# parsakhaz/multimodal-image-similarity-search

Hardware: AMD Instinct MI355X
Metric: images/s CLIP-B/32 encode @ bs256; Mvec/s cosine top-10 over 10M x 512 (higher is better)
Workload: dtype bf16

## Files before the change

multimodal-image-similarity-search_amd/csrc/gemm_bf16_p160.h:

```cpp
#pragma once
#include "gemm_bf16_256.h"

#define G160_A_BYTES 20480
#define G160_W_BYTES 16384
#define G160_BUF (G160_A_BYTES + 2 * G160_W_BYTES)
#define G160_DUMP (3 * G160_BUF)
#define G160_LDS (G160_DUMP + 2048)

template <int EPI, int KT = 0>
__global__ __launch_bounds__(512, 2) void gemm160p_kernel(const __bf16* __restrict__ A, const __bf16* __restrict__ W, int M,
                                                          int N, int K, GemmEpi ep) {
    extern __shared__ __attribute__((aligned(16))) char smem[];
    typedef bf16x8 frag;
    const int tid = threadIdx.x;
    const int lane = tid & 63;
    const int wave = __builtin_amdgcn_readfirstlane(tid >> 6);
    const int wm = wave >> 2, wn = wave & 3;
    const int fr = lane & 15, fg = lane >> 4;
    const int nbm = M / 160, nbn = N >> 8;
    const int nt = KT > 0 ? KT : K / GEMM_BK;
    const int wg = xcd_remap(blockIdx.x, nbm * nbn);
    int bm, bn;
    tile_order(wg, nbm, nbn, 0, bm, bn);
    const __bf16* Ab = A + (size_t)bm * 160 * K;
    const __bf16* Wb = W + (size_t)bn * 256 * K;

    const int r_in = lane >> 3, p = lane & 7;
    const int lane_vo = (r_in * K + ((p ^ r_in) * 8)) * 2;
    const __amdgpu_buffer_rsrc_t srdA = __builtin_amdgcn_make_buffer_rsrc(const_cast<__bf16*>(Ab), 0, 0x7fffffff, 0x00020000);
    const __amdgpu_buffer_rsrc_t srdW = __builtin_amdgcn_make_buffer_rsrc(const_cast<__bf16*>(Wb), 0, 0x7fffffff, 0x00020000);
    const int row8 = 8 * K * 2;
    const int a_so = wave * row8;
    const int a_dst = wave * 1024;
    const int w_so = ((wave >> 1) * 64 + (wave & 1) * 16) * K * 2;
    const int w_dst = wave * 2048;
    char* const dump = smem + G160_DUMP + wave * 256;
#define G160_BLDS(srd, so, dst) \
    __builtin_amdgcn_raw_ptr_buffer_load_lds(srd, (__attribute__((address_space(3))) void*)(dst), 16, lane_vo, so, 0, 0)
#define G160_FILL(srd, so) \
    __builtin_amdgcn_raw_ptr_buffer_load_lds(srd, (__attribute__((address_space(3))) void*)(dump), 4, lane_vo, so, 0, 0)
#define G160_STAGE_A(b2, ko)                                                                                 \
    {                                                                                                       \
        char* sl_ = smem + (b2) * G160_BUF + a_dst;                                                         \
        G160_BLDS(srdA, a_so + (ko), sl_);                                                                  \
        G160_BLDS(srdA, a_so + 8 * row8 + (ko), sl_ + 8 * 1024);                                            \
        if (wave < 4) { G160_BLDS(srdA, a_so + 16 * row8 + (ko), sl_ + 16 * 1024); }                        \
        else { G160_FILL(srdA, a_so + (ko)); }                                                              \
    }
#define G160_STAGE_W(b2, nq, ko)                                                                             \
    {                                                                                                       \
        char* sl_ = smem + (b2) * G160_BUF + G160_A_BYTES + (nq) * G160_W_BYTES + w_dst;                    \
        const int so_ = w_so + (nq) * 4 * row8 + (ko);                                                      \
        G160_BLDS(srdW, so_, sl_);                                                                          \
        G160_BLDS(srdW, so_ + row8, sl_ + 1024);                                                            \
    }

    uint32_t ab[2], wb[2];
#pragma unroll
    for (int s = 0; s < 2; ++s) {
        const uint32_t sw = (((4 * s + fg) ^ (fr & 7)) << 4);
        ab[s] = (wm * 80 + fr) * 128 + sw;
        wb[s] = G160_A_BYTES + (wn * 32 + fr) * 128 + sw;
    }
    frag am[5];
    frag wq[4];
    f32x4 acc[4][5];
#pragma unroll
    for (int i = 0; i < 4; ++i)
#pragma unroll
        for (int j = 0; j < 5; ++j) acc[i][j] = f32x4{0.f, 0.f, 0.f, 0.f};

#define G160_READ(b, s)                                                                                      \
    {                                                                                                       \
        _Pragma("unroll") for (int mf = 0; mf < 5; ++mf)                                                    \
            am[mf] = *reinterpret_cast<const frag*>(smem + ab[s] + (b) * G160_BUF + mf * 2048);             \
        _Pragma("unroll") for (int i = 0; i < 4; ++i)                                                       \
            wq[i] = *reinterpret_cast<const frag*>(smem + wb[s] + (b) * G160_BUF + (i >> 1) * G160_W_BYTES + (i & 1) * 2048); \
    }
#define G160_MMA()                                                                                           \
    {                                                                                                       \
        __builtin_amdgcn_s_setprio(1);                                                                      \
        _Pragma("unroll") for (int i = 0; i < 4; ++i)                                                       \
            _Pragma("unroll") for (int mf = 0; mf < 5; ++mf)                                                \
                acc[i][mf] = __builtin_amdgcn_mfma_f32_16x16x32_bf16(wq[i], am[mf], acc[i][mf], 0, 0, 0);   \
        __builtin_amdgcn_s_setprio(0);                                                                      \
    }
#define G160_BARRIER()                            \
    {                                             \
        __builtin_amdgcn_sched_barrier(0);        \
        __builtin_amdgcn_s_barrier();             \
        __builtin_amdgcn_sched_barrier(0);        \
    }
#define G160_LATE_READS_DONE() \
    if (wm == 1) asm volatile("s_waitcnt lgkmcnt(0)" ::: "memory")
#define G160_KTILE(B, B2)                                                                                    \
    {                                                                                                       \
        G160_READ(B, 0);                                                                                    \
        G160_STAGE_A(B2, ko2);                                                                              \
        G160_LATE_READS_DONE();                                                                             \
        G160_BARRIER();                                                                                     \
        G160_MMA();                                                                                         \
        G160_BARRIER();                                                                                     \
        G160_READ(B, 1);                                                                                    \
        G160_STAGE_W(B2, 0, ko2);                                                                           \
        G160_STAGE_W(B2, 1, ko2);                                                                           \
        G160_LATE_READS_DONE();                                                                             \
        asm volatile("s_waitcnt vmcnt(7)" ::: "memory");                                                    \
        G160_BARRIER();                                                                                     \
        G160_MMA();                                                                                         \
        G160_BARRIER();                                                                                     \
        if (++k2 == nt) { k2 = 0; ko2 = 0; } else { ko2 += GEMM_BK * 2; }                                   \
    }

    constexpr bool RESID = (EPI == MMISS_EPI_BIAS_RESID_BF16);
    static_assert(RESID || EPI == MMISS_EPI_PATCH_F32, "gemm160p_kernel: epilogue");
    u32x2 resid[5][4];
    f32x4 bias[4];
    if constexpr (RESID) {
        const uint16_t* ob = reinterpret_cast<const uint16_t*>(ep.out) + (size_t)(bm * 160 + wm * 80 + fr) * ep.ldo + bn * 256 + wn * 64 + 4 * fg;
#pragma unroll
        for (int j = 0; j < 5; ++j)
#pragma unroll
            for (int i = 0; i < 4; ++i) resid[j][i] = *reinterpret_cast<const u32x2*>(ob + (size_t)j * 16 * ep.ldo + i * 16);
#pragma unroll
        for (int i = 0; i < 4; ++i) bias[i] = *reinterpret_cast<const f32x4*>(ep.bias + bn * 256 + wn * 64 + i * 16 + 4 * fg);
    }

    int ko2 = 0, k2 = 2;
    G160_STAGE_A(0, 0);
    G160_STAGE_W(0, 0, 0);
    G160_STAGE_W(0, 1, 0);
    G160_STAGE_A(1, GEMM_BK * 2);
    G160_STAGE_W(1, 0, GEMM_BK * 2);
    G160_STAGE_W(1, 1, GEMM_BK * 2);
    ko2 = (nt > 2) ? 2 * GEMM_BK * 2 : 0;
    asm volatile("s_waitcnt vmcnt(7)" ::: "memory");
    if constexpr (RESID) {
#pragma unroll
        for (int j = 0; j < 5; ++j)
#pragma unroll
            for (int i = 0; i < 4; ++i) asm volatile("" : "+v"(resid[j][i]));
#pragma unroll
        for (int i = 0; i < 4; ++i) asm volatile("" : "+v"(bias[i]));
    }
    G160_BARRIER();
    if (wm == 1) G160_BARRIER();

#pragma unroll 1
    for (int t = 0; t < nt; t += 3) {
        G160_KTILE(0, 2);
        if (t + 1 < nt) G160_KTILE(1, 0);
        if (t + 2 < nt) G160_KTILE(2, 1);
    }
    if (wm == 0) G160_BARRIER();
    asm volatile("s_waitcnt vmcnt(0)" ::: "memory");
    G160_BARRIER();

    if constexpr (EPI == MMISS_EPI_PATCH_F32) {
        int lane_e = lane;
        asm volatile("" : "+v"(lane_e));
        const int efr = lane_e & 15, efg = lane_e >> 4;
        const int rrow = lane_e >> 3, rchunk = lane_e & 7;
        char* patch = smem + wave * 2048;
        float* outp = reinterpret_cast<float*>(ep.out);
#pragma unroll
        for (int j = 0; j < 5; ++j) {
#pragma unroll
            for (int h = 0; h < 2; ++h) {
#pragma unroll
                for (int ii = 0; ii < 2; ++ii)
                    *reinterpret_cast<f32x4*>(patch + efr * 128 + (((ii * 4 + efg) ^ (efr & 7)) << 4)) = acc[2 * h + ii][j];
                __builtin_amdgcn_fence(__ATOMIC_RELEASE, "wavefront");
                __builtin_amdgcn_wave_barrier();
                __builtin_amdgcn_fence(__ATOMIC_ACQUIRE, "wavefront");
#pragma unroll
                for (int rh = 0; rh < 2; ++rh) {
                    const int row = rh * 8 + rrow;
                    const f32x4 v = *reinterpret_cast<const f32x4*>(patch + row * 128 + ((rchunk ^ (row & 7)) << 4));
                    const int m = bm * 160 + wm * 80 + j * 16 + row;
                    const int n = bn * 256 + wn * 64 + h * 32 + rchunk * 4;
                    if (m < ep.m_valid) {
                        const int img = m / ep.p0, pt = m - img * ep.p0;
                        const f32x4 pos = *reinterpret_cast<const f32x4*>(ep.aux + (size_t)(1 + pt) * ep.ldo + n);
                        *reinterpret_cast<f32x4*>(outp + ((size_t)img * ep.p1 + 1 + pt) * ep.ldo + n) = v + pos;
                    }
                }
                __builtin_amdgcn_wave_barrier();
            }
        }
    }
    if constexpr (RESID) {
        int lane_e = lane;
        asm volatile("" : "+v"(lane_e));
        const int efr = lane_e & 15, efg = lane_e >> 4;
        const int rrow = lane_e >> 3, rchunk = lane_e & 7;
        const __amdgpu_buffer_rsrc_t srdO = __builtin_amdgcn_make_buffer_rsrc(ep.out, 0, 0x7fffffff, 0x00020000);
        char* patch = smem + wave * 2048;
        const int wr_off = efr * 128, wr_sw = 2 * (efr & 7);
        const int col = bn * 256 + wn * 64 + rchunk * 8;
        const int dump_row = M - 1;
#pragma unroll
        for (int j = 0; j < 5; ++j) {
#pragma unroll
            for (int i = 0; i < 4; ++i) {
                const f32x4 v = acc[i][j] + bias[i];
                float y[4];
                y[0] = __uint_as_float(resid[j][i][0] << 16) + v[0];
                y[1] = __uint_as_float(resid[j][i][0] & 0xFFFF0000u) + v[1];
                y[2] = __uint_as_float(resid[j][i][1] << 16) + v[2];
                y[3] = __uint_as_float(resid[j][i][1] & 0xFFFF0000u) + v[3];
                u32x2 pk;
                pk[0] = pack_bf16x2(y[0], y[1]);
                pk[1] = pack_bf16x2(y[2], y[3]);
                *reinterpret_cast<u32x2*>(patch + wr_off + (((i * 4 + efg) ^ wr_sw) << 3)) = pk;
            }
            __builtin_amdgcn_fence(__ATOMIC_RELEASE, "wavefront");
            __builtin_amdgcn_wave_barrier();
            __builtin_amdgcn_fence(__ATOMIC_ACQUIRE, "wavefront");
#pragma unroll
            for (int rh = 0; rh < 2; ++rh) {
                const int row = rh * 8 + rrow;
                const u32x4 pk = *reinterpret_cast<const u32x4*>(patch + row * 128 + (((2 * rchunk) ^ (2 * (row & 7))) << 3));
                const int m = bm * 160 + wm * 80 + j * 16 + row;
                const int vo = ((m < ep.m_valid ? m : dump_row) * ep.ldo + col) * 2;
                __builtin_amdgcn_raw_buffer_store_b128(pk, srdO, vo, 0, 0);
                if (ep.stats_out) {
                    float rs = 0.f, rq = 0.f;
#pragma unroll
                    for (int e = 0; e < 4; ++e) {
                        const float a = __uint_as_float(pk[e] << 16), b = __uint_as_float(pk[e] & 0xFFFF0000u);
                        rs += a + b;
                        rq += a * a + b * b;
                    }
                    rs += __shfl_xor(rs, 1); rq += __shfl_xor(rq, 1);
                    rs += __shfl_xor(rs, 2); rq += __shfl_xor(rq, 2);
                    rs += __shfl_xor(rs, 4); rq += __shfl_xor(rq, 4);
                    if (rchunk == 0 && m < ep.m_valid) {
                        float* so = ep.stats_out + ((size_t)m * (ep.ldo >> 6) + ((bn * 256 + wn * 64) >> 6)) * 2;
                        so[0] = rs;
                        so[1] = rq;
                    }
                }
            }
            __builtin_amdgcn_wave_barrier();
        }
    }
}
#undef G160_BLDS
#undef G160_FILL
#undef G160_STAGE_A
#undef G160_STAGE_W
#undef G160_READ
#undef G160_MMA
#undef G160_BARRIER
#undef G160_LATE_READS_DONE
#undef G160_KTILE

static inline bool gemm160p_ok(int M, int N, int K) {
    if (M <= 0 || (M % 160) || N <= 0 || (N % 256) || K < 256 || (K % 128)) return false;
    if ((int64_t)M * N * 2 >= (1LL << 31) || (int64_t)160 * K * 2 >= (1LL << 31) || (int64_t)256 * K * 2 >= (1LL << 31)) return false;
    return true;
}

static int launch_gemm160p(hipStream_t st, const void* A, const void* W, const GemmEpi& ep, int M, int N, int K) {
    if (!gemm160p_ok(M, N, K)) MM_FAIL(MMISS_ERR_UNSUPPORTED, "gemm160p: M=%d N=%d K=%d", M, N, K);
    if (!ep.out || !ep.bias || ep.ldo < N || (ep.ldo % 64)) MM_FAIL(MMISS_ERR_ARG, "gemm160p: missing operand");
    const int mv = ep.m_valid < M ? ep.m_valid : M;
    const double bytes = 2.0 * ((double)mv * K + (double)N * K) + 2.0 * 2.0 * (double)mv * N;
    char pname[48];
    snprintf(pname, sizeof(pname), "gemm_bf16_bias_resid16_p160_k%d", K);
    MM_PROF(pname, st, 2.0 * mv * N * K, bytes);
#define G160_KT_CASE(KT_)                                                                                                        \
    if (K == (KT_) * GEMM_BK) {                                                                                                  \
        MM_TRY(mmiss_ensure_dyn_lds(reinterpret_cast<const void*>(&gemm160p_kernel<MMISS_EPI_BIAS_RESID_BF16, KT_>), G160_LDS)); \
        hipLaunchKernelGGL((gemm160p_kernel<MMISS_EPI_BIAS_RESID_BF16, KT_>), dim3((M / 160) * (N / 256)), dim3(512), G160_LDS, \
                           st, reinterpret_cast<const __bf16*>(A), reinterpret_cast<const __bf16*>(W), M, N, K, ep);            \
        MM_HIP(hipGetLastError());                                                                                              \
        return MMISS_OK;                                                                                                        \
    }
    G160_KT_CASE(12) G160_KT_CASE(48) G160_KT_CASE(8) G160_KT_CASE(32) G160_KT_CASE(16) G160_KT_CASE(64)
#undef G160_KT_CASE
    MM_TRY(mmiss_ensure_dyn_lds(reinterpret_cast<const void*>(&gemm160p_kernel<MMISS_EPI_BIAS_RESID_BF16>), G160_LDS));
    hipLaunchKernelGGL((gemm160p_kernel<MMISS_EPI_BIAS_RESID_BF16>), dim3((M / 160) * (N / 256)), dim3(512), G160_LDS, st, reinterpret_cast<const __bf16*>(A),
                       reinterpret_cast<const __bf16*>(W), M, N, K, ep);
    MM_HIP(hipGetLastError());
    return MMISS_OK;
}

static int launch_gemm160p_patch(hipStream_t st, const void* A, const void* W, const GemmEpi& ep, int M, int N, int K) {
    if (!gemm160p_ok(M, N, K)) MM_FAIL(MMISS_ERR_UNSUPPORTED, "gemm160p_patch: M=%d N=%d K=%d", M, N, K);
    if (!ep.out || !ep.aux || ep.p0 <= 0 || ep.p1 <= 0 || ep.ldo < N) MM_FAIL(MMISS_ERR_ARG, "gemm160p_patch: missing operand");
    const int mv = ep.m_valid < M ? ep.m_valid : M;
    MM_PROF("gemm_bf16_patch_p160", st, 2.0 * mv * N * K, 2.0 * ((double)mv * K + (double)N * K) + 4.0 * (double)mv * N);
    MM_TRY(mmiss_ensure_dyn_lds(reinterpret_cast<const void*>(&gemm160p_kernel<MMISS_EPI_PATCH_F32>), G160_LDS));
    hipLaunchKernelGGL((gemm160p_kernel<MMISS_EPI_PATCH_F32>), dim3((M / 160) * (N / 256)), dim3(512), G160_LDS, st,
                       reinterpret_cast<const __bf16*>(A), reinterpret_cast<const __bf16*>(W), M, N, K, ep);
    MM_HIP(hipGetLastError());
    return MMISS_OK;
}
```

Measured before the change: 89280.

## Prefetch residual tile via pipelined buffer loads into LDS instead of registers

Instead of loading the bf16 residual tile into VGPRs before the main loop, the last two pipeline prefetch slots are repurposed. Once the K loop wraps, the buffer resources and offsets are retargeted at the output residual rows, so the residual streams into the spare LDS stage buffers via buffer_load_lds. The epilogue then reads the residual from LDS and uses a free stage buffer for its patch staging. This removes 40 held registers across the main loop and overlaps the residual fetch with compute, at the cost of more complex offset bookkeeping and a tight coupling to the 3-stage buffer indexing.

```diff
diff --git a/multimodal-image-similarity-search_amd/csrc/gemm_bf16_p160.h b/multimodal-image-similarity-search_amd/csrc/gemm_bf16_p160.h
--- a/multimodal-image-similarity-search_amd/csrc/gemm_bf16_p160.h
+++ b/multimodal-image-similarity-search_amd/csrc/gemm_bf16_p160.h
@@ -25,15 +25,21 @@
     const __bf16* Ab = A + (size_t)bm * 160 * K;
     const __bf16* Wb = W + (size_t)bn * 256 * K;
 
+    constexpr bool RESID = (EPI == MMISS_EPI_BIAS_RESID_BF16);
+    static_assert(RESID || EPI == MMISS_EPI_PATCH_F32, "gemm160p_kernel: epilogue");
     const int r_in = lane >> 3, p = lane & 7;
-    const int lane_vo = (r_in * K + ((p ^ r_in) * 8)) * 2;
-    const __amdgpu_buffer_rsrc_t srdA = __builtin_amdgcn_make_buffer_rsrc(const_cast<__bf16*>(Ab), 0, 0x7fffffff, 0x00020000);
-    const __amdgpu_buffer_rsrc_t srdW = __builtin_amdgcn_make_buffer_rsrc(const_cast<__bf16*>(Wb), 0, 0x7fffffff, 0x00020000);
+    int lane_vo = (r_in * K + ((p ^ r_in) * 8)) * 2;
+    __amdgpu_buffer_rsrc_t srdA = __builtin_amdgcn_make_buffer_rsrc(const_cast<__bf16*>(Ab), 0, 0x7fffffff, 0x00020000);
+    __amdgpu_buffer_rsrc_t srdW = __builtin_amdgcn_make_buffer_rsrc(const_cast<__bf16*>(Wb), 0, 0x7fffffff, 0x00020000);
     const int row8 = 8 * K * 2;
     const int a_so = wave * row8;
     const int a_dst = wave * 1024;
     const int w_so = ((wave >> 1) * 64 + (wave & 1) * 16) * K * 2;
     const int w_dst = wave * 2048;
+    int xa0 = a_so, xa1 = a_so + 8 * row8, xa2 = a_so + 16 * row8, xaf = a_so;
+    int xw0 = w_so, xw1 = w_so + row8, xw2 = w_so + 4 * row8, xw3 = w_so + 5 * row8;
+    int kstep = GEMM_BK * 2;
+#define G160_X(var, expr) (RESID ? (var) : (expr))
     char* const dump = smem + G160_DUMP + wave * 256;
 #define G160_BLDS(srd, so, dst) \
     __builtin_amdgcn_raw_ptr_buffer_load_lds(srd, (__attribute__((address_space(3))) void*)(dst), 16, lane_vo, so, 0, 0)
@@ -42,18 +48,33 @@
 #define G160_STAGE_A(b2, ko)                                                                                 \
     {                                                                                                       \
         char* sl_ = smem + (b2) * G160_BUF + a_dst;                                                         \
-        G160_BLDS(srdA, a_so + (ko), sl_);                                                                  \
-        G160_BLDS(srdA, a_so + 8 * row8 + (ko), sl_ + 8 * 1024);                                            \
-        if (wave < 4) { G160_BLDS(srdA, a_so + 16 * row8 + (ko), sl_ + 16 * 1024); }                        \
-        else { G160_FILL(srdA, a_so + (ko)); }                                                              \
+        G160_BLDS(srdA, G160_X(xa0, a_so) + (ko), sl_);                                                     \
+        G160_BLDS(srdA, G160_X(xa1, a_so + 8 * row8) + (ko), sl_ + 8 * 1024);                               \
+        if (wave < 4) { G160_BLDS(srdA, G160_X(xa2, a_so + 16 * row8) + (ko), sl_ + 16 * 1024); }           \
+        else { G160_FILL(srdA, G160_X(xaf, a_so) + (ko)); }                                                 \
     }
 #define G160_STAGE_W(b2, nq, ko)                                                                             \
     {                                                                                                       \
         char* sl_ = smem + (b2) * G160_BUF + G160_A_BYTES + (nq) * G160_W_BYTES + w_dst;                    \
-        const int so_ = w_so + (nq) * 4 * row8 + (ko);                                                      \
+        const int so_ = G160_X((nq) ? xw2 : xw0, w_so + (nq) * 4 * row8) + (ko);                            \
         G160_BLDS(srdW, so_, sl_);                                                                          \
-        G160_BLDS(srdW, so_ + row8, sl_ + 1024);                                                            \
-    }
+        G160_BLDS(srdW, G160_X(((nq) ? xw3 : xw1) + (ko), so_ + row8), sl_ + 1024);                         \
+    }
+
+    const int rblk = 16 * ep.ldo * 2;
+    const int lane_vo_r = ((lane >> 2) * ep.ldo + (((lane & 3) ^ (lane >> 4)) * 8)) * 2;
+#define G160_NEXT_KTILE()                                                                                    \
+    if (++k2 == nt) {                                                                                       \
+        if constexpr (RESID) {                                                                              \
+            srdA = srdW = __builtin_amdgcn_make_buffer_rsrc(                                                \
+                reinterpret_cast<uint16_t*>(ep.out) + (size_t)(bm * 160 + wm * 80) * ep.ldo + bn * 256 + wn * 64, 0, 0x7fffffff, \
+                0x00020000);                                                                                \
+            lane_vo = lane_vo_r;                                                                            \
+            xa0 = 0; xa1 = 64; xa2 = 0; xaf = 0;                                                            \
+            xw0 = rblk; xw1 = rblk + 64; xw2 = 2 * rblk; xw3 = 2 * rblk + 64;                               \
+            ko2 = 0; kstep = 2 * rblk;                                                                      \
+        } else { k2 = 0; ko2 = 0; }                                                                         \
+    } else { ko2 += kstep; }
 
     uint32_t ab[2], wb[2];
 #pragma unroll
@@ -109,19 +130,11 @@
         G160_BARRIER();                                                                                     \
         G160_MMA();                                                                                         \
         G160_BARRIER();                                                                                     \
-        if (++k2 == nt) { k2 = 0; ko2 = 0; } else { ko2 += GEMM_BK * 2; }                                   \
-    }
-
-    constexpr bool RESID = (EPI == MMISS_EPI_BIAS_RESID_BF16);
-    static_assert(RESID || EPI == MMISS_EPI_PATCH_F32, "gemm160p_kernel: epilogue");
-    u32x2 resid[5][4];
+        G160_NEXT_KTILE();                                                                                  \
+    }
+
     f32x4 bias[4];
     if constexpr (RESID) {
-        const uint16_t* ob = reinterpret_cast<const uint16_t*>(ep.out) + (size_t)(bm * 160 + wm * 80 + fr) * ep.ldo + bn * 256 + wn * 64 + 4 * fg;
-#pragma unroll
-        for (int j = 0; j < 5; ++j)
-#pragma unroll
-            for (int i = 0; i < 4; ++i) resid[j][i] = *reinterpret_cast<const u32x2*>(ob + (size_t)j * 16 * ep.ldo + i * 16);
 #pragma unroll
         for (int i = 0; i < 4; ++i) bias[i] = *reinterpret_cast<const f32x4*>(ep.bias + bn * 256 + wn * 64 + i * 16 + 4 * fg);
     }
@@ -137,10 +150,6 @@
     asm volatile("s_waitcnt vmcnt(7)" ::: "memory");
     if constexpr (RESID) {
 #pragma unroll
-        for (int j = 0; j < 5; ++j)
-#pragma unroll
-            for (int i = 0; i < 4; ++i) asm volatile("" : "+v"(resid[j][i]));
-#pragma unroll
         for (int i = 0; i < 4; ++i) asm volatile("" : "+v"(bias[i]));
     }
     G160_BARRIER();
@@ -155,13 +164,14 @@
     if (wm == 0) G160_BARRIER();
     asm volatile("s_waitcnt vmcnt(0)" ::: "memory");
     G160_BARRIER();
+    const int free_buf = RESID ? ((nt + 2) % 3) * G160_BUF : 0;
 
     if constexpr (EPI == MMISS_EPI_PATCH_F32) {
         int lane_e = lane;
         asm volatile("" : "+v"(lane_e));
         const int efr = lane_e & 15, efg = lane_e >> 4;
         const int rrow = lane_e >> 3, rchunk = lane_e & 7;
-        char* patch = smem + wave * 2048;
+        char* patch = smem + free_buf + wave * 2048;
         float* outp = reinterpret_cast<float*>(ep.out);
 #pragma unroll
         for (int j = 0; j < 5; ++j) {
@@ -195,10 +205,25 @@
         const int efr = lane_e & 15, efg = lane_e >> 4;
         const int rrow = lane_e >> 3, rchunk = lane_e & 7;
         const __amdgpu_buffer_rsrc_t srdO = __builtin_amdgcn_make_buffer_rsrc(ep.out, 0, 0x7fffffff, 0x00020000);
-        char* patch = smem + wave * 2048;
+        char* patch = smem + free_buf + wave * 2048;
         const int wr_off = efr * 128, wr_sw = 2 * (efr & 7);
         const int col = bn * 256 + wn * 64 + rchunk * 8;
         const int dump_row = M - 1;
+        u32x2 resid[5][4];
+        {
+            const char* const st0 = smem + (nt % 3) * G160_BUF;
+            const char* const st1 = smem + ((nt + 1) % 3) * G160_BUF;
+            const int rd = efr * 64 + ((((efg >> 1) ^ (efr >> 2)) << 4) | ((efg & 1) << 3));
+#pragma unroll
+            for (int j = 0; j < 5; ++j)
+#pragma unroll
+                for (int i = 0; i < 4; ++i) {
+                    const int h = i >> 1;
+                    const char* piece = j == 0 ? st0 + a_dst + h * 8 * 1024
+                                               : (j < 3 ? st0 : st1) + G160_A_BYTES + ((j - 1) & 1) * G160_W_BYTES + w_dst + h * 1024;
+                    resid[j][i] = *reinterpret_cast<const u32x2*>(piece + (rd ^ ((i & 1) << 5)));
+                }
+        }
 #pragma unroll
         for (int j = 0; j < 5; ++j) {
 #pragma unroll
@@ -255,6 +280,8 @@
 #undef G160_BARRIER
 #undef G160_LATE_READS_DONE
 #undef G160_KTILE
+#undef G160_NEXT_KTILE
+#undef G160_X
 
 static inline bool gemm160p_ok(int M, int N, int K) {
     if (M <= 0 || (M % 160) || N <= 0 || (N % 256) || K < 256 || (K % 128)) return false;
```

Measured after the change: 91490 (median of 6 runs). 2.5% higher.
